# anonymous-author-918/deq-mpc-corl

Hardware: AMD Instinct MI355X
Metric: QP solves/sec at (B,T=20,nx=13,nu=4) (higher is better)
Workload: dtype f32

## Files before the change

### deq-mpc-corl_amd/csrc/alqp_quad.hip

```cpp
#if defined(ALQP_BWD_DYN_UNIT) || defined(ALQP_SHDYN_UNIT)
#undef ALQP_PHASE_TIMING
#endif
#include <hip/hip_runtime.h>

#include "alqp_quad.hpp"
#include "alqp_dims.hpp"
#include "alqp_launch.hpp"

#if defined(ALQP_QUAD_F32) == defined(ALQP_QUAD_F64)
#error "compile alqp_quad.hip with exactly one of -DALQP_QUAD_F32, -DALQP_QUAD_F64"
#endif

namespace alqp {

#ifndef ALQP_FUSE_LS
#define ALQP_FUSE_LS 1
#endif
#ifdef ALQP_PHASE_TIMING
__device__ unsigned long long g_phase_cycles[10];
#define QSTAMP(b) qd.stamp(b)
#else
#define QSTAMP(b)
#endif
#ifdef ALQP_SHDYN_UNIT
template <typename real, int NX, int NU, bool TRACE, class Dyn = NoDyn>
__global__ __launch_bounds__(64) __attribute__((amdgpu_waves_per_eu(1, 1))) void k_solve_lin_quad_shdyn(ShdynSolveArgs<real> a, TraceArgs<real> tr, real *ws) {
#else
template <typename real, int NX, int NU, bool TRACE, class Dyn = NoDyn>
__global__ __launch_bounds__(64) __attribute__((amdgpu_waves_per_eu(1, 1))) void k_solve_lin_quad(SolveArgs<real> a, TraceArgs<real> tr, real *ws) {
#endif
    using C = QCfg<real, NX, NU>;
    constexpr bool NL = Dyn::ID != 0;
#ifndef ALQP_FUSE_LS_F64
#define ALQP_FUSE_LS_F64 1
#endif
    constexpr bool FUSE_LS = ALQP_FUSE_LS && (sizeof(real) == 4 || ALQP_FUSE_LS_F64) && !NL;
    constexpr int N = C::N;
    if (a.skip && *a.skip != 0.0) return;
    const int lane = threadIdx.x, qi = lane >> 2;
    const int b_raw = blockIdx.x * 16 + qi;
    const bool active = b_raw < a.B;
    {
        int stag = a.stagger;
        const int mode = (a.flags >> 20) & 0xf;
        if ((a.flags >> 24) & 0xff) stag = (a.flags >> 24) & 0xff;
        if (stag > 0) {
            const unsigned hw = __builtin_amdgcn_s_getreg(4 | (0 << 6) | (31 << 11));
            int simd = (hw >> 4) & 3;
            if (mode == 1) simd = simd * 16 + ((hw >> 8) & 0xf);
            if (mode == 2) simd &= 1;
            if (mode == 3) simd = blockIdx.x & 1;
            if (mode == 4) simd = (simd & 1) ^ (blockIdx.x & 1);
            if (mode == 5) simd = (hw >> 8) & 3;
            for (int i = 0; i < simd * stag; ++i) __builtin_amdgcn_s_sleep(16);
        }
    }
#ifdef ALQP_ALIAS_ALL
    const int b = (active ? b_raw : a.B - 1) % ALQP_ALIAS_ALL;
#else
    const int b = active ? b_raw : a.B - 1;
#endif
    const int T = a.T, M = C::M(T);

    Quad<real, NX, NU> qd;
    __shared__ real w_lds[QCfg<real, NX, NU>::WLDS_WORDS];
    qd.wl = w_lds + threadIdx.x;
    constexpr bool FL = C::KL > 0;
    if constexpr (FL) {
        __shared__ __attribute__((aligned(16))) real l_lds[C::KL * C::FLW];
        qd.fl = (ALQP_LDS real *)l_lds;
        qd.kl = (a.flags & ALQP_FACTOR_IN_WS) ? 0 : (T < C::KL ? T : C::KL);
    }
    qd.q = lane & 3;
    qd.T = T;
    qd.active = active;
    qd.gQd = a.Qd + (size_t)b * T * N;
    qd.gq = a.q + (size_t)b * T * N;
#ifdef ALQP_SHDYN_UNIT
    qd.gF = a.F + (size_t)b * a.sb_F;
    qd.gc = a.c + (size_t)b * a.sb_c;
    qd.mt_F = a.mt_F; qd.mt_c = a.mt_c;
#else
    qd.gF = a.F + (size_t)b * (T - 1) * NX * N;
    qd.gc = a.c + (size_t)b * (T - 1) * NX;
#endif
    qd.gx0 = a.x0 + (size_t)b * NX;
    qd.gulo = a.ulo + (size_t)b * a.sb_u;
    qd.guhi = a.uhi + (size_t)b * a.sb_u;
    qd.st_u = a.st_u;
    qd.gz = a.z + (size_t)b * T * N;
    qd.glam = a.lam + (size_t)b * M;
    qd.rec = ws + C::rec_base(b, T);
    qd.gFw = const_cast<real *>(qd.gF);
    qd.dyn_h = a.dyn_h;
    qd.rho = a.rho[b];
    qd.info = 0;
    real phi_prev = a.phi[b];
#ifdef ALQP_PHASE_TIMING
    for (int i = 0; i < 10; ++i) qd.tacc[i] = 0;
#endif
    QSTAMP(-1);
    if (!(a.flags & ALQP_WS_PRIMED)) {
        if constexpr (NL) qd.stage_in(false, false);
        else qd.stage_in(a.max_newton == 0 || a.al_iter == 0 || (a.flags & ALQP_EXIT_IN_KERNEL) ||
                         (!C::PHI0_FWD && (a.flags & ALQP_INIT_MERIT)));
    }
    const bool ref_exit = (a.flags & ALQP_EXIT_IN_KERNEL) != 0;
    int gphase = 0;

    int step_id = 0;
    bool pend = false;
    real alpha_pend = 0;
    int bad = 0;
    real rn2 = 0, phi_next = 0;
    for (int it = 0; it < a.al_iter; ++it) {
        bool phi_from_forward = false;
        if (a.flags & ALQP_INIT_MERIT) {
            if (it > 0) {
                phi_prev = phi_next;
            } else if (C::PHI0_FWD && a.max_newton > 0 && !ref_exit) {
                phi_from_forward = true;
            } else {
                if constexpr (NL) qd.template linearize<Dyn>(real(0), false);
                real p1[1];
                qd.template merit_candidates<1>(p1, true);
                phi_prev = p1[0];
            }
        }
        pend = false;
        double nrm_old = 0;
        int n_done = 0;
        if (ref_exit) {
            int bad0 = 0;
            const real r0 = it == 0 ? qd.rplus2(bad0) : rn2;
            nrm_old = sqrt(grid_sum_ordered(wave_sum_leaders(exit_term(r0, qor(qd.info)), active && qd.q == 0), a.exit_scratch, gphase));
        }
        for (int st = 0; st < a.max_newton; ++st, ++step_id) {
            real *tg = nullptr;
            if constexpr (TRACE) tg = (tr.g && active) ? tr.g + ((size_t)step_id * a.B + b) * T * N : nullptr;
            QSTAMP(9);
            if constexpr (NL) {
                qd.template linearize<Dyn>(alpha_pend, pend);
                pend = false;
            }
            if constexpr (FL) qd.fl_ws = ref_exit || (it + 1 == a.al_iter && st + 1 == a.max_newton);
            qd.template forward<false, FL>(tg, alpha_pend, pend, (phi_from_forward && st == 0) ? &phi_prev : nullptr);
            real ph[20];
            const bool store_s = !FUSE_LS || ref_exit || st + 1 == a.max_newton;
            qd.template backward<FUSE_LS, FL>(ph, nullptr, store_s);
            QSTAMP(-1);
            if constexpr (TRACE) {
                if (tr.d && active) {
                    real *td = tr.d + ((size_t)step_id * a.B + b) * T * N;
                    for (int t = 0; t < T; ++t)
                        for (int j = qd.q; j < N; j += 4) td[t * N + j] = qd.recp(t)[C::wn(C::oY, j)];
                }
            }
            if constexpr (NL) qd.template merit_nonlin<Dyn>(ph);
            else if constexpr (!FUSE_LS) qd.template merit_candidates<20>(ph, false);
            QSTAMP(6);
            int kbest = 0;
            real best = ph[0];
#pragma unroll
            for (int k = 1; k < 20; ++k) {
                if (k < a.n_ls && !(best != best) && (ph[k] != ph[k] || ph[k] < best)) {
                    best = ph[k];
                    kbest = k;
                }
            }
            const bool acc = best < phi_prev;
            if constexpr (TRACE) {
                if (active && qd.q == 0) {
                    if (tr.phi)
#pragma unroll
                        for (int k = 0; k < 20; ++k)
                            if (k < a.n_ls) tr.phi[((size_t)step_id * a.n_ls + k) * a.B + b] = ph[k];
                    if (tr.phi_prev) tr.phi_prev[(size_t)step_id * a.B + b] = phi_prev;
                    if (tr.k) tr.k[(size_t)step_id * a.B + b] = kbest;
                    if (tr.accept) tr.accept[(size_t)step_id * a.B + b] = acc ? 1 : 0;
                }
            }
            const real alpha = acc ? real(1) / real(1 << kbest) : real(0);
            pend = true;
            alpha_pend = alpha;
            QSTAMP(7);
            phi_prev = best;
            if (ref_exit) {
                int bad1 = 0;
                real ph_unused = 0, r1 = 0;
                qd.template iter_end<Dyn>(alpha_pend, pend, false, (real)a.rho_scale, false, ph_unused, r1, bad1);
                pend = false;
                const double nw = sqrt(grid_sum_ordered(wave_sum_leaders(exit_term(r1, qor(qd.info)), active && qd.q == 0), a.exit_scratch, gphase));
                ++n_done;
                if (nw < a.exit_tol || fabs(nrm_old - nw) / nw < a.exit_tol) break;
                nrm_old = nw;
            }
        }
        if (ref_exit && a.newton_counts && blockIdx.x == 0 && lane == 0) a.newton_counts[it] = grid_barrier_timed_out(a.exit_scratch) ? -1 : n_done;
        bad = 0;
        qd.template iter_end<Dyn>(alpha_pend, pend, (a.flags & ALQP_DUAL_UPDATE) != 0, (real)a.rho_scale, it + 1 == a.al_iter,
                    phi_next, rn2, bad);
        pend = false;
    }
    if (a.al_iter <= 0) {
        rn2 = qd.rplus2(bad);
        qd.stage_out();
    }
#ifdef ALQP_PHASE_TIMING
    QSTAMP(9);
    if (lane == 0)
        for (int i = 0; i < 10; ++i) atomicAdd(&g_phase_cycles[i], qd.tacc[i]);
#endif
    if (active && qd.q == 0) {
        a.rho[b] = qd.rho;
        a.phi[b] = phi_prev;
        if (a.rnorm2) a.rnorm2[b] = rn2;
        if (a.info && qd.info && a.info[b] == 0) a.info[b] = qd.info;
        if (a.status) a.status[b] = bad ? 0 : 1;
    }
}

template <typename real, int NX, int NU, bool DYN = false>
__global__ __launch_bounds__(64) __attribute__((amdgpu_waves_per_eu(1, 1))) void k_backward_quad(BwdArgs<real, DYN> a, real *ws) {
    using C = QCfg<real, NX, NU>;
    constexpr int N = C::N;
    const int lane = threadIdx.x, qi = lane >> 2;
    const int b_raw = blockIdx.x * 16 + qi;
    const bool active = b_raw < a.B;
    const int b = active ? b_raw : a.B - 1;
    const int T = a.T;
    Quad<real, NX, NU> qd;
    __shared__ real w_lds[QCfg<real, NX, NU>::WLDS_WORDS];
// ... 201 lines not shown
```

### deq-mpc-corl_amd/csrc/alqp_quad.hpp

```cpp
#pragma once
#include <hip/hip_runtime.h>

#include <type_traits>

#include "alqp_team.hpp"
#include "alqp_dyn.hpp"

namespace alqp {

template <int Q>
__device__ inline float qb(float v) {
    return __builtin_bit_cast(float, __builtin_amdgcn_mov_dpp(__builtin_bit_cast(int, v), Q * 0x55, 0xF, 0xF, true));
}
template <int Q>
__device__ inline double qb(double v) {
    long long b = __builtin_bit_cast(long long, v);
    int lo = __builtin_amdgcn_mov_dpp((int)(b & 0xffffffffll), Q * 0x55, 0xF, 0xF, true);
    int hi = __builtin_amdgcn_mov_dpp((int)(b >> 32), Q * 0x55, 0xF, 0xF, true);
    return __builtin_bit_cast(double, ((long long)hi << 32) | (unsigned int)lo);
}
template <typename real>
__device__ inline real qbv(real v, int src) {
    switch (src & 3) {
        case 0: return qb<0>(v);
// ... 100 lines not shown
template <int LEN, typename real>
__device__ __forceinline__ void gload(const real *p, WRowLds<real, LEN> row) {
    real tmp[LEN];
    gload<LEN>(p, tmp);
#pragma unroll
    for (int k = 0; k < LEN; ++k) row[k] = tmp[k];
}

struct NoDyn {
    static constexpr int ID = 0;
};

struct Fld {
    int h, t;
};
template <int H, int T>
struct FldT {
    static constexpr int h = H, t = T;
    __host__ __device__ constexpr operator Fld() const { return {H, T}; }
};
template <typename real>
struct FRef {
    real *p;
    Fld f;
};
template <typename real, int H, int T>
__device__ __forceinline__ FRef<std::remove_const_t<real>> operator+(real *p, FldT<H, T>) {
    return {const_cast<std::remove_const_t<real> *>(p), Fld{H, T}};
}

template <typename real, int NX_, int NU_>
struct QCfg {
    static constexpr int NX = NX_, NU = NU_, N = NX_ + NU_;
    static constexpr int SH = (N + 3) / 4;
    static constexpr int SW = (NX + 3) / 4;
    static constexpr int SY = SH;
    static constexpr int HT = 2 * SH * (SH + 1);
    __host__ __device__ static constexpr int hidx(int s, int j) { return 2 * s * (s + 1) + j; }
    static constexpr int ST = 2 * SW * (SW + 1);
    static constexpr int BLK = 64 / (int)sizeof(real);
#ifndef ALQP_REC_IL_F32
#define ALQP_REC_IL_F32 2
#endif
    static constexpr int IL = sizeof(real) == 4 ? ALQP_REC_IL_F32 : 1;
    static_assert(IL == 1 || BLK == 16, "groups of 16 words are 64-byte blocks");
    __host__ __device__ static constexpr int w(int x) { return (x / 16) * (16 * IL) + x % 16; }
    static constexpr int NLAST = N - 4 * (SH - 1);
    __host__ __device__ static constexpr int lanes_of(int s) { return s == SH - 1 ? NLAST : 4; }
    __host__ __device__ static constexpr int lstride(int s) { return lanes_of(s) == 3 ? 16 : 4 * lanes_of(s); }
    __host__ __device__ static constexpr int lbase(int s) {
        int o = 0;
        for (int i = 0; i < s; ++i) o += (i + 1) * lstride(i);
        return o;
    }
    static constexpr int LW = lbase(SH);
    static constexpr bool PHI0_FWD = sizeof(real) == 4;
#ifndef ALQP_S_AFTER_F32
#define ALQP_S_AFTER_F32 0
#endif
    static constexpr bool S_AFTER = sizeof(real) == 8 || ALQP_S_AFTER_F32;
#ifndef ALQP_W_LDS_F32
#define ALQP_W_LDS_F32 0
#endif
    static constexpr bool W_LDS = ALQP_W_LDS && (sizeof(real) == 8 || ALQP_W_LDS_F32);
    static constexpr int WLDS_WORDS = W_LDS ? SW * N * 64 : 1;
#ifndef ALQP_PANEL_OWNER_SCALE
#define ALQP_PANEL_OWNER_SCALE 1
#endif
#ifndef ALQP_PANEL_OWNER_SCALE_F64
#define ALQP_PANEL_OWNER_SCALE_F64 ALQP_PANEL_OWNER_SCALE
#endif
    static constexpr bool OWNER_SCALE = sizeof(real) == 8 ? ALQP_PANEL_OWNER_SCALE_F64 : ALQP_PANEL_OWNER_SCALE;
    __host__ __device__ static constexpr int fl_chunk(int s) { return 16 * 4 * lanes_of(s); }
    __host__ __device__ static constexpr int fl_base(int s) {
        int o = 0;
        for (int i = 0; i < s; ++i) o += (i + 1) * fl_chunk(i);
        return o;
    }
    static constexpr int FLW = fl_base(SH);
    static constexpr int FL_BUDGET = 36 * 1024 / 4;
#ifndef ALQP_FACTOR_LDS_F32
#define ALQP_FACTOR_LDS_F32 -1
#endif
    static constexpr int KL = (sizeof(real) != 4 || W_LDS) ? 0
                              : ALQP_FACTOR_LDS_F32 >= 0   ? ALQP_FACTOR_LDS_F32
                              : N > 17                     ? 0
                              : (FL_BUDGET / FLW < 8 ? FL_BUDGET / FLW : 8);
    static_assert(KL * FLW <= 40 * 1024 / 4, "four wavefronts' factor stages fit a CU's LDS");
    __host__ __device__ static constexpr int p4(int x) { return (x + 3) & ~3; }
    static constexpr int NF = 9;
    __host__ __device__ static constexpr int fslots(int i) { return (i <= 1 || i == 6 || i == 7) ? SY : (i == 5 ? 4 : SW); }
    static constexpr int oL = 2 * 16 * (SY / 4);
    __host__ __device__ static constexpr int tail_at(int i) {
        int g = (oL + LW + 15) & ~15, o = 0;
        for (int k = 0; k < NF; ++k) {
            const int r = fslots(k) % 4;
            if (r > 0 && o + r > 4) { g += 16; o = 0; }
            if (k == i) return g + o;
            o += r;
        }
        return o > 0 ? g + 16 : g;
    }
    __host__ __device__ static constexpr int head_at(int i) {
        if (i < 2) return i * 16 * (SY / 4);
        int o = tail_at(NF);
        for (int k = 2; k < i; ++k) o += 16 * (fslots(k) / 4);
        return o;
    }
    static constexpr FldT<head_at(0), tail_at(0)> oY{};
    static constexpr FldT<head_at(1), tail_at(1)> oZ{};
    static constexpr FldT<head_at(2), tail_at(2)> oR{};
    static constexpr FldT<head_at(3), tail_at(3)> oS{};
    static constexpr FldT<head_at(4), tail_at(4)> oLE{};
    static_assert(NU <= 4, "the u-slot layout holds one control per lane");
    static constexpr FldT<head_at(5), tail_at(5)> oUS{};
    static constexpr FldT<head_at(6), tail_at(6)> oQ{};
    static constexpr FldT<head_at(7), tail_at(7)> oq{};
    static constexpr FldT<head_at(8), tail_at(8)> oC{};
    static constexpr int RECW = (head_at(NF) + 31) & ~31;
    static_assert(IL == 1 || RECW % 16 == 0, "whole groups per record");
    template <int S>
    __host__ __device__ static constexpr int lp(int m, int q) {
        return m < 4 * (S / 4) ? 16 * (m / 4) + 4 * q + m % 4 : 16 * (S / 4) + q * (S % 4) + m - 4 * (S / 4);
    }
    template <int S>
    __host__ __device__ static constexpr int fw(Fld f, int p) {
        return p < 16 * (S / 4) ? w(f.h + p) : w(f.t + 4 * ((p - 16 * (S / 4)) / (S % 4)) + (p - 16 * (S / 4)) % (S % 4));
    }
    __host__ __device__ static constexpr int pn(int k) { return lp<SY>(k >> 2, k & 3); }
    __host__ __device__ static constexpr int px(int r) { return lp<SW>(r >> 2, r & 3); }
    __host__ __device__ static constexpr int wn(Fld f, int k) { return fw<SY>(f, pn(k)); }
    __host__ __device__ static constexpr int M(int T) { return T * NX + 2 * T * NU; }
    static constexpr int RSTR = RECW * IL;
    __host__ __device__ static constexpr size_t rec_base(int b, int T) { return (size_t)(b / IL) * T * RSTR + (size_t)(b % IL) * 16; }
    __host__ __device__ static constexpr size_t ws_words(int B, int T) { return (size_t)((B + IL - 1) / IL) * T * RSTR; }
    __host__ static bool ws_covers(int B, int T) {
        return rec_base(B - 1, T) + (size_t)(T - 1) * RSTR + w(RECW - 1) + 1 <= ws_words(B, T);
    }
};

template <typename real, int NX, int NU>
struct Quad {
    using C = QCfg<real, NX, NU>;
    static constexpr int N = C::N, SH = C::SH, SW = C::SW, SY = C::SY, HT = C::HT, ST = C::ST, RECW = C::RECW;

    int q, T;
    bool active;
    const real *gQd, *gq, *gF, *gc, *gx0, *gulo, *guhi;
    long st_u;
#ifdef ALQP_SHDYN_UNIT
    int mt_F, mt_c;
#endif
    real *gz, *glam, *rec;
    real rho;
    int info;
    real *wl;
    using WT = WPanel<real, SW, N, C::W_LDS>;
    __device__ __forceinline__ WT wpanel() const {
        if constexpr (C::W_LDS) return WT{wl};
        else return WT{};
    }
    real *gFw;
    real dyn_h;
    const real *gobs;
    int nobs;
    real obs_r2;
    bool no_init;
    ALQP_LDS real *fl;
    int kl;
    bool fl_ws;
    __device__ __forceinline__ void fstage(int t, ALQP_LDS real *&pl, ALQP_LDS real *&pc) const {
        int lane;
        asm volatile("v_mbcnt_lo_u32_b32 %0, -1, 0\n\tv_mbcnt_hi_u32_b32 %0, -1, %0" : "=v"(lane));
        pl = fl + t * C::FLW + 4 * lane;
        pc = fl + t * C::FLW + 4 * C::NLAST * (lane >> 2);
    }
    __device__ __forceinline__ ALQP_LDS real *fchunk(ALQP_LDS real *pl, ALQP_LDS real *pc, int s, int c, int ql) const {
        return (C::lanes_of(s) == 4 ? pl : pc + 4 * ql) + C::fl_base(s) + c * C::fl_chunk(s);
    }
    __device__ __forceinline__ void st_factor_ws(real *rp, const real (&H)[HT]) const {
#pragma unroll
        for (int s = 0; s < SH; ++s)
#pragma unroll
            for (int c = 0; c <= s; ++c)
                if (C::lanes_of(s) == 4 || q < C::lanes_of(s))
                    gst4(lchunk(rp, s, c, q), H[C::hidx(s, 4 * c)],
                         H[C::hidx(s, 4 * c + 1)], H[C::hidx(s, 4 * c + 2)], H[C::hidx(s, 4 * c + 3)]);
    }
    __device__ __forceinline__ void st_factor_lds(int t, const real (&H)[HT]) const {
        ALQP_LDS real *pl, *pc;
        fstage(t, pl, pc);
#pragma unroll
        for (int s = 0; s < SH; ++s)
#pragma unroll
            for (int c = 0; c <= s; ++c)
                if (C::lanes_of(s) == 4 || q < C::lanes_of(s))
                    lst4<real>(fchunk(pl, pc, s, c, q), H[C::hidx(s, 4 * c)],
                         H[C::hidx(s, 4 * c + 1)], H[C::hidx(s, 4 * c + 2)], H[C::hidx(s, 4 * c + 3)]);
    }
    __device__ __forceinline__ void ld_factor_ws(real *rp, real (&H)[HT]) const {
#pragma unroll
        for (int s = 0; s < SH; ++s)
#pragma unroll
            for (int c = 0; c <= s; ++c) {
                const int ql = (C::lanes_of(s) == 4 || q < C::lanes_of(s)) ? q : 0;
                gld4(lchunk(rp, s, c, ql), H[C::hidx(s, 4 * c)],
                     H[C::hidx(s, 4 * c + 1)], H[C::hidx(s, 4 * c + 2)], H[C::hidx(s, 4 * c + 3)]);
            }
    }
    __device__ __forceinline__ void ld_factor_lds(int t, real (&H)[HT]) const {
        ALQP_LDS real *pl, *pc;
        fstage(t, pl, pc);
#pragma unroll
        for (int s = 0; s < SH; ++s)
#pragma unroll
            for (int c = 0; c <= s; ++c) {
                const int ql = (C::lanes_of(s) == 4 || q < C::lanes_of(s)) ? q : 0;
                lld4<real>(fchunk(pl, pc, s, c, ql), H[C::hidx(s, 4 * c)],
                     H[C::hidx(s, 4 * c + 1)], H[C::hidx(s, 4 * c + 2)], H[C::hidx(s, 4 * c + 3)]);
            }
    }

    __device__ __forceinline__ real uhi(int t, int j) const { return guhi[t * st_u + j]; }
    __device__ __forceinline__ real ulo(int t, int j) const { return gulo[t * st_u + j]; }
    __device__ __forceinline__ real *recp(int t) const { return rec + (size_t)t * C::RSTR; }
#ifdef ALQP_PHASE_TIMING
    unsigned long long tacc[10], tlast;
    __device__ __forceinline__ void stamp(int bucket) {
        unsigned long long now;
        __builtin_amdgcn_sched_barrier(0);
        asm volatile("s_waitcnt vmcnt(0)\n\ts_memtime %0\n\ts_waitcnt lgkmcnt(0)" : "=s"(now)::"memory");
        __builtin_amdgcn_sched_barrier(0);
        if (bucket >= 0) tacc[bucket] += now - tlast;
        tlast = now;
    }
#define ALQP_STAMP(b) stamp(b)
#else
#define ALQP_STAMP(b)
#endif

    template <int S, int L>
    __device__ __forceinline__ void ld_slots(FRef<real> f, real (&v)[L]) const {
        static_assert(L <= S, "slots of the field");
#pragma unroll
        for (int c = 0; 4 * c < L && c < S / 4; ++c) {
            const real *p = f.p + C::w(f.f.h + 16 * c) + 4 * q;
            if (4 * c + 3 < L) gld4(p, v[4 * c], v[4 * c + 1], v[4 * c + 2], v[4 * c + 3]);
            else
#pragma unroll
                for (int i = 0; 4 * c + i < L; ++i) v[4 * c + i] = p[i];
        }
        constexpr int H = 4 * (S / 4), R = S % 4;
        if constexpr (L > H) {
            const real *p = f.p + C::w(f.f.t) + 4 * q;
#pragma unroll
            for (int m = H; m < L; ++m) v[m] = p[m - H];
        }
    }
// ... 283 lines not shown
                    co[s] = okr ? c : real(0);
                    ro[s] = okr ? zn[s] - xr : real(0);
                }
                if (active) {
                    st_own_x(rp + C::oC, co);
                    st_own_x(rp + C::oR, ro);
                }
            }
        }
    }
    template <class Dyn>
    __device__ __forceinline__ void merit_nonlin(real (&phi)[20]) {
        real m[5];
#pragma unroll
        for (int i = 0; i < 5; ++i) m[i] = 0;
        real x0v[NX], li[NX];
        gload<NX>(gx0, x0v);
        ld_rep_x(recp(T - 1) + C::oLE, li);
        const real a0 = sel4(real(1), real(0.5), real(0.25), real(0.125), q);
        for (int t = 0; t < T; ++t) {
            const bool dyn = t < T - 1;
            const real *rp = recp(t), *rn = recp(dyn ? t + 1 : t);
            real zt[N], dt[N], Qt[N], qt[N], zn[NX], dn[NX], le[NX], lu[NU], ll[NU], bu[NU], bl[NU];
            ld_rep_n(rp + C::oZ, zt);
            ld_rep_n(rp + C::oY, dt);
            ld_rep_n(rp + C::oQ, Qt);
            ld_rep_n(rp + C::oq, qt);
            ld_repx_of_n(rn + C::oZ, zn);
            ld_repx_of_n(rn + C::oY, dn);
            ld_rep_x(rp + C::oLE, le);
            ld_rep_us(rp, lu, ll, bu, bl);
            real alpha = a0;
#pragma unroll
            for (int i = 0; i < 5; ++i) {
                real zc[N];
                real acc = 0;
#pragma unroll
                for (int j = 0; j < N; ++j) {
                    zc[j] = fma_(alpha, dt[j], zt[j]);
                    acc = fma_(fma_(real(0.5) * Qt[j], zc[j], qt[j]), zc[j], acc);
                }
#pragma unroll
                for (int ju = 0; ju < NU; ++ju) {
                    const real vu = zc[NX + ju] - bu[ju], vl = bl[ju] - zc[NX + ju];
                    const real cu = fmax_(vu, real(0)), cl = fmax_(vl, real(0));
                    acc += fma_(lu[ju], vu, ll[ju] * vl) + real(0.5) * rho * fma_(cu, cu, cl * cl);
                }
                if (dyn) {
                    real xn[NX];
                    dyn_value<Dyn, real>(zc, dyn_h, xn);
#pragma unroll
                    for (int r = 0; r < NX; ++r) {
                        const real rr = fma_(alpha, dn[r], zn[r]) - xn[r];
                        acc = fma_(fma_(real(0.5) * rho, rr, le[r]), rr, acc);
                    }
                }
                if (t == 0) {
#pragma unroll
                    for (int r = 0; r < NX; ++r) {
                        const real rr = zc[r] - x0v[r];
                        acc = fma_(fma_(real(0.5) * rho, rr, li[r]), rr, acc);
                    }
                }
                m[i] += acc;
                alpha *= real(0.0625);
            }
        }
#pragma unroll
        for (int k = 0; k < 20; ++k) phi[k] = qbv(m[k >> 2], k);
    }

    template <int NHS>
    __device__ __forceinline__ static real panel_mult(const real (&H)[HT], const real (&hs)[NHS], real ip, int j, int k) {
        if constexpr (C::OWNER_SCALE) return qbv(hs[k >> 2], k);
        else return qbv(H[C::hidx(k >> 2, j)], k) * ip;
    }
    __device__ __forceinline__ static real pcol(real a) {
        if constexpr (C::OWNER_SCALE) return a;
        else return -a;
    }

    template <bool EXT = false, bool FL = false>
    __device__ __forceinline__ void forward(real *g_out, real alpha, bool pending, real *phi0, const real *gxn = nullptr) {
        real mdist = 0;
        real S[ST], Sy[SW];
        real vpo[SW], Syo[SW];
        real zc[SW];
#pragma unroll
        for (int i = 0; i < ST; ++i) S[i] = 0;
#pragma unroll
        for (int s = 0; s < SW; ++s) Sy[s] = 0;
        {
            real z0[SW], xi[SW], li[SW], r0[SW];
            if constexpr (EXT) {
                ld_own_ext<NX>(gz, z0);
                ld_own_ext<NX>(glam + (T - 1) * NX, li);
            } else {
                ld_ownx_of_n(recp(0) + C::oZ, z0);
                ld_own_x(recp(T - 1) + C::oLE, li);
            }
            ld_own_ext<NX>(gx0, xi);
            if (pending) {
                real d0[SW];
                ld_ownx_of_n(recp(0) + C::oY, d0);
#pragma unroll
                for (int s = 0; s < SW; ++s) z0[s] = fma_(alpha, d0[s], z0[s]);
            }
#pragma unroll
            for (int s = 0; s < SW; ++s) {
                bool valid = 4 * s + 3 < NX || 4 * s + q < NX;
                if constexpr (EXT) valid = valid && !no_init;
                const real r = valid ? z0[s] - xi[s] : real(0);
                vpo[s] = valid ? fma_(rho, r, li[s]) : real(0);
                if constexpr (C::PHI0_FWD) mdist += valid ? fma_(fma_(real(0.5) * rho, r, li[s]), r, real(0)) : real(0);
                Syo[s] = 0;
                r0[s] = r;
                zc[s] = z0[s];
            }
            if (!EXT && active) st_own_x(recp(T - 1) + C::oR, r0);
        }
        for (int t = 0; t < T; ++t) {
            const bool dyn = t < T - 1;
            WT W = wpanel();
            real Y[N];
            real dio[SY];
            real v[SW];
            real zs[SY];
            real hob[3] = {0, 0, 0};
            real *rp = recp(t);
            {
                real zt[N];
                real Qo[SY], qo[SY];
                real cs[SW], zn[SW], lm[SW];
                real lu, ll, bu, bl;
                const int td = dyn ? t : (T > 1 ? T - 2 : 0);
                const real *rn = recp(td + 1);
                if constexpr (EXT) {
                    ld_own_ext<N>(gz + t * N, zs);
                    ld_own_ext<N>(gQd + t * N, Qo);
                    ld_own_ext<N>(gq + t * N, qo);
                    load_F_rows(td, W);
                    ld_own_ext<NX>(gxn + td * NX, cs);
                    ld_own_ext<NX>(gz + (td + 1) * N, zn);
                    ld_own_ext<NX>(glam + td * NX, lm);
                    const int ju = own_ju(), jc = ju < NU ? ju : 0;
                    const real *lb = glam + T * NX + t * (2 * NU + nobs);
                    const bool has = ju < NU;
                    lu = has ? lb[jc] : real(0);
                    ll = has ? lb[NU + jc] : real(0);
                    bu = has ? guhi[t * st_u + jc] : real(0);
                    bl = has ? gulo[t * st_u + jc] : real(0);
                } else {
#pragma unroll
                    for (int s = 0; s < SW; ++s) zs[s] = zc[s];
                    ld_slots_from<SY, SW>(rp + C::oZ, zs);
                    if constexpr (ALQP_EXP_NOQ) { for (int m = 0; m < SY; ++m) Qo[m] = real(1); }
                    else ld_own_n(rp + C::oQ, Qo);
                    ld_own_n(rp + C::oq, qo);
                    load_F_rows(td, W);
                    ld_own_x(rp + C::oC, cs);
                    ld_ownx_of_n(rn + C::oZ, zn);
                    ld_own_x(rp + C::oLE, lm);
                    ld_own_us(rp, lu, ll, bu, bl);
                }
                if (pending) {
                    real dt[SY], dn[SW];
                    constexpr int M0 = EXT ? 0 : SW;
                    ld_slots_from<SY, M0>(rp + C::oY, dt);
                    ld_ownx_of_n(rn + C::oY, dn);
#pragma unroll
                    for (int m = M0; m < SY; ++m) zs[m] = fma_(alpha, dt[m], zs[m]);
#pragma unroll
                    for (int s = 0; s < SW; ++s) zn[s] = fma_(alpha, dn[s], zn[s]);
                }
#pragma unroll
                for (int s = 0; s < SW; ++s) zc[s] = zn[s];
                ALQP_STAMP(0);
#pragma unroll
                for (int k = 0; k < N; ++k) zt[k] = qbv(zs[k >> 2], k);
                real rro[SW];
                if (!dyn) {
#pragma unroll
                    for (int s = 0; s < SW; ++s)
#pragma unroll
                        for (int k = 0; k < N; ++k) W[s][k] = 0;
                }
#pragma unroll
                for (int s = 0; s < SW; ++s) {
                    const int r = 4 * s + q;
                    real xn = cs[s];
                    if constexpr (!EXT) {
#pragma unroll
                        for (int k = 0; k < N; ++k) xn = fma_(W[s][k], zt[k], xn);
                    }
                    const real rr = zn[s] - xn;
                    const bool ok = dyn && r < NX;
                    v[s] = ok ? fma_(rho, rr, lm[s]) : real(0);
                    rro[s] = ok ? rr : real(0);
                    if constexpr (C::PHI0_FWD) mdist += ok ? fma_(fma_(real(0.5) * rho, rr, lm[s]), rr, real(0)) : real(0);
                }
                if (!ALQP_EXP_NORS && !EXT && dyn && active) st_own_x(rp + C::oR, rro);
                constexpr int MU0 = NX / 4;
                real zu = 0;
#pragma unroll
                for (int m = MU0; m < SY; ++m) zu = (4 * m + q >= NX && 4 * m + q < N) ? zs[m] : zu;
                const real vu = zu - bu, vl = bl - zu;
                const real au = vu >= 0 ? real(1) : real(0), al = vl >= 0 ? real(1) : real(0);
                const real cu = fmax_(vu, real(0)), cl = fmax_(vl, real(0));
                const real gu = fma_(rho, cu, lu) - fma_(rho, cl, ll);
                const real du = rho * (au + al);
                if constexpr (C::PHI0_FWD)
                    mdist += own_ju() < NU ? fma_(lu, vu, ll * vl) + real(0.5) * rho * fma_(cu, cu, cl * cl) : real(0);
                real go[SY];
#pragma unroll
                for (int m = 0; m < SY; ++m) {
                    const int j = 4 * m + q;
                    const bool isx = (4 * m + 3 < NX) ? true : (4 * m >= NX ? false : j < NX);
                    const bool isu = (4 * m + 3 < NX) ? false : (j >= NX && j < N);
                    real g = fma_(Qo[m], zs[m], qo[m]);
                    real d = Qo[m];
                    if constexpr (C::PHI0_FWD) mdist = fma_(fma_(real(0.5) * Qo[m], zs[m], qo[m]), zs[m], mdist);
                    g += isx ? vpo[m < SW ? m : 0] : (isu ? gu : real(0));
                    bool pinned = isx;
                    if constexpr (EXT) {
                        pinned = isx && !(no_init && t == 0);
                        if (no_init && isu) g = 0;
                    }
                    d += pinned ? rho : (isu ? du : real(0));
                    dio[m] = d;
                    go[m] = g;
                }
                if constexpr (EXT && NX >= 3) {
                    if (nobs > 0) {
                        const real *lk = glam + T * NX + t * (2 * NU + nobs) + 2 * NU;
                        real gob = 0;
                        for (int k = 0; k < nobs; ++k) {
                            const real *o = gobs + (size_t)(t * nobs + k) * 3;
                            const real d0 = zt[0] - o[0], d1 = zt[1] - o[1], d2 = zt[2] - o[2];
                            const real ck = obs_r2 - fma_(d0, d0, fma_(d1, d1, d2 * d2));
                            const real dh = q == 0 ? d0 : (q == 1 ? d1 : d2);
                            gob = fma_(fma_(rho, ck > 0 ? ck : real(0), lk[k]), real(-2) * dh, gob);
                            if (ck >= 0) {
                                const real w4 = real(4) * rho * dh;
                                hob[0] = fma_(w4, d0, hob[0]); hob[1] = fma_(w4, d1, hob[1]); hob[2] = fma_(w4, d2, hob[2]);
                            }
                        }
                        go[0] += q < 3 ? gob : real(0);
                    }
                }
#pragma unroll
                for (int m = 0; m < SY; ++m) {
                    const bool isx = (4 * m + 3 < NX) ? true : (4 * m >= NX ? false : 4 * m + q < NX);
// ... 62 lines not shown
                    for (int s = 0; s < SH; ++s) {
                        real fi = sel4(fr[4 * s], (4 * s + 1 < N) ? fr[(4 * s + 1 < N) ? 4 * s + 1 : 0] : real(0),
                                       (4 * s + 2 < N) ? fr[(4 * s + 2 < N) ? 4 * s + 2 : 0] : real(0),
                                       (4 * s + 3 < N) ? fr[(4 * s + 3 < N) ? 4 * s + 3 : 0] : real(0), q) * irho;
#pragma unroll
                        for (int j = 0; j < 4 * s + 4; ++j)
                            if (j < N) H[C::hidx(s, j)] = fma_(fi, fr[j], H[C::hidx(s, j)]);
                    }
                }
            }
            ALQP_STAMP(1);
            real ipv[C::S_AFTER ? N : 1];
#pragma unroll
            for (int j = 0; j < N; ++j) {
                const real p = qbv(H[C::hidx(j >> 2, j)], j);
                if (!(p > 0) && info == 0) info = t * N + j + 1;
                const real ip = rcp_(fabs_(p));
                real hs[C::OWNER_SCALE ? SH : 1];
                if constexpr (C::OWNER_SCALE) {
                    const real nip = -ip;
#pragma unroll
                    for (int m = (j >> 2); m < SH; ++m) hs[m] = H[C::hidx(m, j)] * nip;
                }
                if constexpr (C::W_LDS) {
                    constexpr int KB = 8;
                    real wj[SW];
#pragma unroll
                    for (int s = 0; s < SW; ++s) wj[s] = W[s][j];
#pragma unroll
                    for (int k0 = j + 1; k0 < N; k0 += KB) {
                        real wv[KB][SW];
#pragma unroll
                        for (int kk = 0; kk < KB; ++kk)
#pragma unroll
                            for (int s = 0; s < SW; ++s)
                                if (k0 + kk < N) wv[kk][s] = W[s][k0 + kk];
                        __builtin_amdgcn_sched_barrier(0);
#pragma unroll
                        for (int kk = 0; kk < KB; ++kk) {
                            const int k = k0 + kk;
                            if (k < N) {
                                const real lkj = panel_mult(H, hs, ip, j, k);
#pragma unroll
                                for (int s = (k >> 2); s < SH; ++s) H[C::hidx(s, k)] = fma_(pcol(H[C::hidx(s, j)]), lkj, H[C::hidx(s, k)]);
#pragma unroll
                                for (int s = 0; s < SW; ++s) W[s][k] = fma_(pcol(wj[s]), lkj, wv[kk][s]);
                                Y[k] = fma_(pcol(Y[j]), lkj, Y[k]);
                            }
                        }
                    }
                } else {
#pragma unroll
                for (int k = j + 1; k < N; ++k) {
                    const real lkj = panel_mult(H, hs, ip, j, k);
#pragma unroll
                    for (int s = (k >> 2); s < SH; ++s) H[C::hidx(s, k)] = fma_(pcol(H[C::hidx(s, j)]), lkj, H[C::hidx(s, k)]);
#pragma unroll
                    for (int s = 0; s < SW; ++s) W[s][k] = fma_(pcol(W[s][j]), lkj, W[s][k]);
                    Y[k] = fma_(pcol(Y[j]), lkj, Y[k]);
                }
                }
                if constexpr (C::S_AFTER) ipv[j] = ip;
                if (!C::S_AFTER && dyn) {
                    real wsc[C::OWNER_SCALE ? SW : 1];
                    if constexpr (C::OWNER_SCALE) {
#pragma unroll
                        for (int s = 0; s < SW; ++s) wsc[s] = W[s][j] * ip;
                    }
#pragma unroll
                    for (int b = 0; b < NX; ++b) {
                        real wbj;
                        if constexpr (C::OWNER_SCALE) wbj = qbv(wsc[b >> 2], b);
                        else wbj = qbv(W[b >> 2][j], b) * ip;
#pragma unroll
                        for (int s = (b >> 2); s < SW; ++s) S[C::hidx(s, b)] = fma_(W[s][j], wbj, S[C::hidx(s, b)]);
                    }
                    const real yip = Y[j] * ip;
#pragma unroll
                    for (int s = 0; s < SW; ++s) Sy[s] = fma_(W[s][j], yip, Sy[s]);
                }
                H[C::hidx(j >> 2, j)] = (q == (j & 3)) ? ip : H[C::hidx(j >> 2, j)];
            }
            ALQP_STAMP(2);
            if (active) {
                if constexpr (FL) {
                    if (t >= kl || fl_ws) st_factor_ws(rp, H);
                } else
                if (!(ALQP_EXP_NOL && t >= T - ALQP_EXP_NOL))
#pragma unroll
                for (int s = 0; s < SH; ++s)
#pragma unroll
                    for (int c = 0; c <= s; ++c)
                        if (C::lanes_of(s) == 4 || q < C::lanes_of(s))
                            gst4(lchunk(rp, s, c, q), H[C::hidx(s, 4 * c)],
                                 H[C::hidx(s, 4 * c + 1)], H[C::hidx(s, 4 * c + 2)], H[C::hidx(s, 4 * c + 3)]);
                real yo[SY];
                own_of<N, SY>(Y, yo);
                st_own_n(rp + C::oY, yo);
                if (pending) st_own_n(rp + C::oZ, zs);
            }
            if constexpr (FL) {
                if (t < kl) st_factor_lds(t, H);
            }

            if constexpr (C::S_AFTER) {
                if (dyn) {
#pragma unroll
                    for (int j = 0; j < N; ++j) {
                        real wsc[C::OWNER_SCALE ? SW : 1];
                        if constexpr (C::OWNER_SCALE) {
#pragma unroll
                            for (int s = 0; s < SW; ++s) wsc[s] = W[s][j] * ipv[j];
                        }
#pragma unroll
                        for (int b = 0; b < NX; ++b) {
                            real wbj;
                            if constexpr (C::OWNER_SCALE) wbj = qbv(wsc[b >> 2], b);
                            else wbj = qbv(W[b >> 2][j], b) * ipv[j];
#pragma unroll
                            for (int s = (b >> 2); s < SW; ++s) S[C::hidx(s, b)] = fma_(W[s][j], wbj, S[C::hidx(s, b)]);
                        }
                        const real yip = Y[j] * ipv[j];
#pragma unroll
                        for (int s = 0; s < SW; ++s) Sy[s] = fma_(W[s][j], yip, Sy[s]);
                    }
                }
            }
#pragma unroll
            for (int s = 0; s < SW; ++s) {
                vpo[s] = v[s];
                Syo[s] = Sy[s];
            }
            ALQP_STAMP(3);
        }
        if constexpr (C::PHI0_FWD) { if (phi0) *phi0 = qsum(mdist); }
    }

    __host__ __device__ static constexpr int lane_lo(int m, int j) { return m == (j >> 2) ? (j & 3) + 1 : 0; }
    __device__ __forceinline__ bool in_lanes(int lo, int hi) const {
        return lo == 0 ? q < hi : (hi == 4 ? q >= lo : (q >= lo && q < hi));
    }
    __device__ __forceinline__ void lsolve_own(const real (&H)[HT], real (&u)[SY]) const {
#pragma unroll
        for (int j = 0; j < N; ++j) {
            const int mj = j >> 2;
            const real wj = qbv(u[mj] * H[C::hidx(mj, j)], j);
#pragma unroll
            for (int m = mj; m < SH; ++m) {
                const int lo = lane_lo(m, j);
                if (lo >= C::lanes_of(m)) continue;
                const real v = fma_(-H[C::hidx(m, j)], wj, u[m]);
                u[m] = lo == 0 ? v : (q >= lo ? v : u[m]);
            }
        }
    }
    __device__ __forceinline__ void ltsolve_own(const real (&H)[HT], const real (&y)[SY], real (&d)[SY], real (&rep)[N]) const {
#pragma unroll
        for (int m = 0; m < SY; ++m) d[m] = 0;
#pragma unroll
        for (int i = N - 1; i >= 0; --i) {
            const int mi = i >> 2;
            real p = 0;
            bool any = false;
#pragma unroll
            for (int m = mi; m < SH; ++m) {
                const int lo = lane_lo(m, i), hi = C::lanes_of(m);
                if (lo >= hi) continue;
                const real h = (lo == 0 && hi == 4) ? H[C::hidx(m, i)] : (in_lanes(lo, hi) ? H[C::hidx(m, i)] : real(0));
                p = any ? fma_(h, d[m], p) : h * d[m];
                any = true;
            }
            real r = y[mi];
            if (any) r -= qsum(p);
            const real di = qbv(r * H[C::hidx(mi, i)], i);
            rep[i] = di;
            d[mi] = (q == (i & 3)) ? di : d[mi];
        }
    }

    template <bool LS, bool FL = false>
    __device__ __forceinline__ void backward(real (&phi)[20], real *d_ext = nullptr, bool store_s = true) {
        constexpr int MU0 = NX / 4;
        real c0 = 0, c1 = 0, c2 = 0;
        real acc[20];
        real rvT[SW], lvT[SW];
#pragma unroll
        for (int k = 0; k < 20; ++k) acc[k] = 0;
#pragma unroll
        for (int s = 0; s < SW; ++s) rvT[s] = lvT[s] = 0;
        real dxs[SW];
#pragma unroll
        for (int s = 0; s < SW; ++s) dxs[s] = 0;
        for (int t = T - 1; t >= 0; --t) {
            const bool dyn = t < T - 1;
            real *rp = recp(t);
            real H[HT];
            if constexpr (FL) {
                static_assert(!FL || !ALQP_EXP_NOL, "the no-factor experiment runs with the factor in the records");
                if (t < kl) ld_factor_lds(t, H);
                else ld_factor_ws(rp, H);
            } else
            if (ALQP_EXP_NOL && t >= T - ALQP_EXP_NOL) {
#pragma unroll
                for (int i = 0; i < HT; ++i) H[i] = real(1);
            } else
#pragma unroll
            for (int s = 0; s < SH; ++s)
#pragma unroll
                for (int c = 0; c <= s; ++c) {
                    const int ql = (C::lanes_of(s) == 4 || q < C::lanes_of(s)) ? q : 0;
                    gld4(lchunk(rp, s, c, ql), H[C::hidx(s, 4 * c)],
                         H[C::hidx(s, 4 * c + 1)], H[C::hidx(s, 4 * c + 2)], H[C::hidx(s, 4 * c + 3)]);
                }
            real yo[SY];
            ld_own_n(rp + C::oY, yo);
            WT W = wpanel();
            load_F_rows(dyn ? t : (T > 1 ? T - 2 : 0), W);
            real zz[SY], QQ[SY], qq[SY], rv[SW], lv[SW];
            real lu = 0, ll = 0, bu = 0, bl = 0;
            if constexpr (LS) {
                ld_own_n(rp + C::oZ, zz);
                if constexpr (ALQP_EXP_NOQ) { for (int m = 0; m < SY; ++m) QQ[m] = real(1); }
                else ld_own_n(rp + C::oQ, QQ);
                ld_own_n(rp + C::oq, qq);
                ld_own_us(rp, lu, ll, bu, bl);
                if constexpr (ALQP_EXP_NORS) { for (int s = 0; s < SW; ++s) rv[s] = real(0); }
                else ld_own_x(rp + C::oR, rv);
                ld_own_x(rp + C::oLE, lv);
            }
            ALQP_STAMP(4);
            if (dyn) {
                real vv[N];
#pragma unroll
                for (int j = 0; j < N; ++j) {
                    real p = 0;
#pragma unroll
                    for (int s = 0; s < SW; ++s) p = fma_(W[s][j], dxs[s], p);
                    vv[j] = qsum(p);
                }
                real uo[SY];
                own_of<N, SY>(vv, uo);
                lsolve_own(H, uo);
#pragma unroll
                for (int m = 0; m < SY; ++m) yo[m] = fma_(rho, uo[m], yo[m]);
            }
            real down[SY], Y[N];
            ltsolve_own(H, yo, down, Y);
            if (active) {
                if (d_ext) st_own_ext<N>(d_ext + t * N, down);
                else st_own_n(rp + C::oY, down);
            }
            real sv[SW];
#pragma unroll
            for (int s = 0; s < SW; ++s) sv[s] = 0;
            if (dyn) {
#pragma unroll
                for (int s = 0; s < SW; ++s) {
                    const int r = 4 * s + q;
                    real p = 0;
#pragma unroll
                    for (int k = 0; k < N; ++k) p = fma_(W[s][k], Y[k], p);
                    sv[s] = (4 * s + 3 < NX || r < NX) ? dxs[s] - p : real(0);
                }
                if (!ALQP_EXP_NORS && active && !d_ext && store_s) st_own_x(rp + C::oS, sv);
            }
            if constexpr (LS) {
                real zu = 0, du = 0;
#pragma unroll
                for (int m = 0; m < SY; ++m) {
                    const int j = 4 * m + q;
                    const real ok = (4 * m + 3 < N || j < N) ? real(1) : real(0);
                    const real z = zz[m], d = down[m], Qv = QQ[m] * ok, qv = qq[m] * ok;
                    c0 = fma_(fma_(real(0.5) * Qv, z, qv), z, c0);
                    c1 = fma_(fma_(Qv, z, qv), d, c1);
                    c2 = fma_(real(0.5) * Qv * d, d, c2);
                    if (m >= MU0) {
                        const bool mine = j >= NX && j < N;
                        zu = mine ? z : zu;
                        du = mine ? d : du;
                    }
                }
                {
                    const real isu = own_ju() < NU ? real(1) : real(0);
                    real alpha = 1;
#pragma unroll
                    for (int k = 0; k < 20; ++k) {
                        real zk = fma_(alpha, du, zu);
                        real vu = zk - bu, vl = bl - zk;
                        real cu = fmax_(vu, real(0)), cl = fmax_(vl, real(0));
                        acc[k] = fma_(isu, fma_(lu, vu, ll * vl) + real(0.5) * rho * fma_(cu, cu, cl * cl), acc[k]);
                        alpha *= real(0.5);
                    }
                }
                if (dyn) {
#pragma unroll
                    for (int s = 0; s < SW; ++s) {
                        const int r = 4 * s + q;
                        const real ok = (4 * s + 3 < NX || r < NX) ? real(1) : real(0);
                        const real rr = rv[s] * ok, ss = sv[s] * ok, lm = lv[s] * ok;
                        c0 = fma_(fma_(real(0.5) * rho, rr, lm), rr, c0);
                        c1 = fma_(fma_(rho, rr, lm), ss, c1);
                        c2 = fma_(real(0.5) * rho * ss, ss, c2);
                    }
                } else {
#pragma unroll
                    for (int s = 0; s < SW; ++s) {
                        rvT[s] = rv[s];
                        lvT[s] = lv[s];
                    }
                }
            }
#pragma unroll
            for (int s = 0; s < SW; ++s) dxs[s] = (4 * s + 3 < NX || 4 * s + q < NX) ? down[s] : real(0);
            ALQP_STAMP(5);
        }
        if (active && !d_ext && store_s) st_own_x(recp(T - 1) + C::oS, dxs);
        if constexpr (LS) {
#pragma unroll
            for (int s = 0; s < SW; ++s) {
                const int r = 4 * s + q;
                const real ok = (4 * s + 3 < NX || r < NX) ? real(1) : real(0);
                const real rr = rvT[s] * ok, ss = dxs[s], lm = lvT[s] * ok;
                c0 = fma_(fma_(real(0.5) * rho, rr, lm), rr, c0);
                c1 = fma_(fma_(rho, rr, lm), ss, c1);
                c2 = fma_(real(0.5) * rho * ss, ss, c2);
            }
            c0 = qsum(c0);
            c1 = qsum(c1);
            c2 = qsum(c2);
            real alpha = 1;
// ... 272 lines not shown
```

Baseline: 6.808 million.

## Stage per-stage y/d vectors in LDS alongside factor stages for N=17

Adds an LDS staging area for the forward solve's y vector and the backward solve's step d, used for the first KD time stages when N==17. It shrinks the factor LDS stage count by one to make room. Forward and backward then read and write these vectors from LDS instead of global workspace records, and the global d store is skipped unless it is needed for the last step or for tracing. This trades global memory round trips for LDS capacity and one fewer factor stage held in LDS.

Result: slower. 6.637 million (-2.5%).

```diff
diff --git a/deq-mpc-corl_amd/csrc/alqp_quad.hip b/deq-mpc-corl_amd/csrc/alqp_quad.hip
--- a/deq-mpc-corl_amd/csrc/alqp_quad.hip
+++ b/deq-mpc-corl_amd/csrc/alqp_quad.hip
@@ -67,9 +67,13 @@
     qd.wl = w_lds + threadIdx.x;
     constexpr bool FL = C::KL > 0;
     if constexpr (FL) {
-        __shared__ __attribute__((aligned(16))) real l_lds[C::KL * C::FLW];
+        __shared__ __attribute__((aligned(16))) real l_lds[C::KL * C::FLW + C::KD * C::YDW];
         qd.fl = (ALQP_LDS real *)l_lds;
         qd.kl = (a.flags & ALQP_FACTOR_IN_WS) ? 0 : (T < C::KL ? T : C::KL);
+        if constexpr (C::KD > 0) {
+            qd.yl = (ALQP_LDS real *)l_lds + C::KL * C::FLW;
+            qd.kd = (a.flags & ALQP_FACTOR_IN_WS) ? 0 : (T < C::KD ? T : C::KD);
+        }
     }
     qd.q = lane & 3;
     qd.T = T;
@@ -147,7 +151,8 @@
             qd.template forward<false, FL>(tg, alpha_pend, pend, (phi_from_forward && st == 0) ? &phi_prev : nullptr);
             real ph[20];
             const bool store_s = !FUSE_LS || ref_exit || st + 1 == a.max_newton;
-            qd.template backward<FUSE_LS, FL>(ph, nullptr, store_s);
+            if constexpr (C::KD > 0) qd.template backward<FUSE_LS, FL>(ph, nullptr, store_s, store_s || TRACE);
+            else qd.template backward<FUSE_LS, FL>(ph, nullptr, store_s);
             QSTAMP(-1);
             if constexpr (TRACE) {
                 if (tr.d && active) {
diff --git a/deq-mpc-corl_amd/csrc/alqp_quad.hpp b/deq-mpc-corl_amd/csrc/alqp_quad.hpp
--- a/deq-mpc-corl_amd/csrc/alqp_quad.hpp
+++ b/deq-mpc-corl_amd/csrc/alqp_quad.hpp
@@ -206,11 +206,30 @@
 #ifndef ALQP_FACTOR_LDS_F32
 #define ALQP_FACTOR_LDS_F32 -1
 #endif
+    static constexpr int YDW = SY * 64;
+    static constexpr int LDS_CAP = 40 * 1024 / 4;
+#ifndef ALQP_YD_LDS_F32
+#define ALQP_YD_LDS_F32 -1
+#endif
+#ifdef ALQP_SHDYN_UNIT
+    static constexpr bool YD_SPLIT = false;
+#else
+    static constexpr bool YD_SPLIT = N == 17;
+#endif
     static constexpr int KL = (sizeof(real) != 4 || W_LDS) ? 0
                               : ALQP_FACTOR_LDS_F32 >= 0   ? ALQP_FACTOR_LDS_F32
                               : N > 17                     ? 0
+                              : (YD_SPLIT && ALQP_YD_LDS_F32 < 0) ? FL_BUDGET / FLW - 1
                               : (FL_BUDGET / FLW < 8 ? FL_BUDGET / FLW : 8);
-    static_assert(KL * FLW <= 40 * 1024 / 4, "four wavefronts' factor stages fit a CU's LDS");
+    static constexpr int KD = KL == 0                ? 0
+                              : ALQP_YD_LDS_F32 >= 0 ? ALQP_YD_LDS_F32
+                              : !YD_SPLIT            ? 0
+                              : ((LDS_CAP - KL * FLW) / YDW < 20 ? (LDS_CAP - KL * FLW) / YDW : 20);
+    static_assert(KL * FLW + KD * YDW <= LDS_CAP, "four wavefronts' factor and y/d stages fit a CU's LDS");
+#ifndef ALQP_YD_ITEMS
+#define ALQP_YD_ITEMS 3
+#endif
+    static constexpr bool YD_Y = KD > 0 && (ALQP_YD_ITEMS & 1), YD_D = KD > 0 && (ALQP_YD_ITEMS & 2);
     __host__ __device__ static constexpr int p4(int x) { return (x + 3) & ~3; }
     static constexpr int NF = 9;
     __host__ __device__ static constexpr int fslots(int i) { return (i <= 1 || i == 6 || i == 7) ? SY : (i == 5 ? 4 : SW); }
@@ -298,6 +317,42 @@
         asm volatile("v_mbcnt_lo_u32_b32 %0, -1, 0\n\tv_mbcnt_hi_u32_b32 %0, -1, %0" : "=v"(lane));
         pl = fl + t * C::FLW + 4 * lane;
         pc = fl + t * C::FLW + 4 * C::NLAST * (lane >> 2);
+    }
+    ALQP_LDS real *yl;
+    int kd;
+    __device__ __forceinline__ static int yd_lane() {
+        int lane;
+        asm volatile("v_mbcnt_lo_u32_b32 %0, -1, 0\n\tv_mbcnt_hi_u32_b32 %0, -1, %0" : "=v"(lane));
+        return lane;
+    }
+    __device__ __forceinline__ ALQP_LDS real *yd_stage(int t) const {
+        asm volatile("" : "+s"(t));
+        return yl + t * C::YDW;
+    }
+    template <int L0, int L1, int LEN>
+    __device__ __forceinline__ void ld_yd_lds(int t, int lane, real (&v)[LEN]) const {
+        static_assert(L0 >= 0 && L0 <= L1 && L1 <= SY && L1 <= LEN, "slots of the field");
+        constexpr int HC = SY / 4;
+        const ALQP_LDS real *ps = yd_stage(t);
+#pragma unroll
+        for (int c = L0 / 4; c < HC && 4 * c < L1; ++c) {
+            real w[4];
+            lld4<real>(ps + 256 * c + 4 * lane, w[0], w[1], w[2], w[3]);
+#pragma unroll
+            for (int i = 0; i < 4; ++i)
+                if (4 * c + i >= L0 && 4 * c + i < L1) v[4 * c + i] = w[i];
+        }
+#pragma unroll
+        for (int m = (L0 > 4 * HC ? L0 : 4 * HC); m < L1; ++m) v[m] = ps[64 * m + lane];
+    }
+    __device__ __forceinline__ void st_yd_lds(int t, const real (&v)[SY]) const {
+        constexpr int HC = SY / 4;
+        const int lane = yd_lane();
+        ALQP_LDS real *ps = yd_stage(t);
+#pragma unroll
+        for (int c = 0; c < HC; ++c) lst4<real>(ps + 256 * c + 4 * lane, v[4 * c], v[4 * c + 1], v[4 * c + 2], v[4 * c + 3]);
+#pragma unroll
+        for (int m = 4 * HC; m < SY; ++m) ps[64 * m + lane] = v[m];
     }
     __device__ __forceinline__ ALQP_LDS real *fchunk(ALQP_LDS real *pl, ALQP_LDS real *pc, int s, int c, int ql) const {
         return (C::lanes_of(s) == 4 ? pl : pc + 4 * ql) + C::fl_base(s) + c * C::fl_chunk(s);
@@ -747,6 +802,7 @@
 
     template <bool EXT = false, bool FL = false>
     __device__ __forceinline__ void forward(real *g_out, real alpha, bool pending, real *phi0, const real *gxn = nullptr) {
+        constexpr bool YD = FL && C::YD_Y, YDD = FL && C::YD_D;
         real mdist = 0;
         real S[ST], Sy[SW];
         real vpo[SW], Syo[SW];
@@ -767,6 +823,10 @@
             ld_own_ext<NX>(gx0, xi);
             if (pending) {
                 real d0[SW];
+                if constexpr (YDD) {
+                    if (kd > 0) ld_yd_lds<0, SW>(0, yd_lane(), d0);
+                    else ld_ownx_of_n(recp(0) + C::oY, d0);
+                } else
                 ld_ownx_of_n(recp(0) + C::oY, d0);
 #pragma unroll
                 for (int s = 0; s < SW; ++s) z0[s] = fma_(alpha, d0[s], z0[s]);
@@ -831,8 +891,16 @@
                 if (pending) {
                     real dt[SY], dn[SW];
                     constexpr int M0 = EXT ? 0 : SW;
+                    if constexpr (YDD) {
+                        const int lane = yd_lane();
+                        if (t < kd) ld_yd_lds<M0, SY>(t, lane, dt);
+                        else ld_slots_from<SY, M0>(rp + C::oY, dt);
+                        if (td + 1 < kd) ld_yd_lds<0, SW>(td + 1, lane, dn);
+                        else ld_ownx_of_n(rn + C::oY, dn);
+                    } else {
                     ld_slots_from<SY, M0>(rp + C::oY, dt);
                     ld_ownx_of_n(rn + C::oY, dn);
+                    }
 #pragma unroll
                     for (int m = M0; m < SY; ++m) zs[m] = fma_(alpha, dt[m], zs[m]);
 #pragma unroll
@@ -1061,6 +1129,8 @@
                 H[C::hidx(j >> 2, j)] = (q == (j & 3)) ? ip : H[C::hidx(j >> 2, j)];
             }
             ALQP_STAMP(2);
+            real yo[SY];
+            if constexpr (YD) own_of<N, SY>(Y, yo);
             if (active) {
                 if constexpr (FL) {
                     if (t >= kl || fl_ws) st_factor_ws(rp, H);
@@ -1073,10 +1143,12 @@
                         if (C::lanes_of(s) == 4 || q < C::lanes_of(s))
                             gst4(lchunk(rp, s, c, q), H[C::hidx(s, 4 * c)],
                                  H[C::hidx(s, 4 * c + 1)], H[C::hidx(s, 4 * c + 2)], H[C::hidx(s, 4 * c + 3)]);
-                real yo[SY];
-                own_of<N, SY>(Y, yo);
-                st_own_n(rp + C::oY, yo);
+                if constexpr (!YD) own_of<N, SY>(Y, yo);
+                if (!YD || t >= kd) st_own_n(rp + C::oY, yo);
                 if (pending) st_own_n(rp + C::oZ, zs);
+            }
+            if constexpr (YD) {
+                if (t < kd) st_yd_lds(t, yo);
             }
             if constexpr (FL) {
                 if (t < kl) st_factor_lds(t, H);
@@ -1158,7 +1230,8 @@
     }
 
     template <bool LS, bool FL = false>
-    __device__ __forceinline__ void backward(real (&phi)[20], real *d_ext = nullptr, bool store_s = true) {
+    __device__ __forceinline__ void backward(real (&phi)[20], real *d_ext = nullptr, bool store_s = true, bool store_d = true) {
+        constexpr bool YD = FL && C::YD_Y, YDD = FL && C::YD_D;
         constexpr int MU0 = NX / 4;
         real c0 = 0, c1 = 0, c2 = 0;
         real acc[20];
@@ -1192,6 +1265,10 @@
                          H[C::hidx(s, 4 * c + 1)], H[C::hidx(s, 4 * c + 2)], H[C::hidx(s, 4 * c + 3)]);
                 }
             real yo[SY];
+            if constexpr (YD) {
+                if (t < kd) ld_yd_lds<0, SY>(t, yd_lane(), yo);
+                else ld_own_n(rp + C::oY, yo);
+            } else
             ld_own_n(rp + C::oY, yo);
             WT W = wpanel();
             load_F_rows(dyn ? t : (T > 1 ? T - 2 : 0), W);
@@ -1225,6 +1302,10 @@
             }
             real down[SY], Y[N];
             ltsolve_own(H, yo, down, Y);
+            if constexpr (YDD) {
+                if (active && (t >= kd || store_d)) st_own_n(rp + C::oY, down);
+                if (t < kd) st_yd_lds(t, down);
+            } else
             if (active) {
                 if (d_ext) st_own_ext<N>(d_ext + t * N, down);
                 else st_own_n(rp + C::oY, down);
```
